# hip-satomi/microbeSEG

Measured on AMD Instinct MI355X. Metric: training crops/sec (256px), higher is better.
Workload: dtype f32; 1 GPU; BASELINE configs[1]: DU-Net distance-map training step, filters [64, 1024], 256x256 crops, per-GPU batch 32, fp32, relu/bn, SmoothL1x2 + Adam(amsgrad); global_batch=32, parallelism=dp1, launch=eager

## Files before the change

### include/mseg_hip.h

```cpp
#ifndef MSEG_HIP_H
#define MSEG_HIP_H

#include <stddef.h>
#include <stdint.h>

#ifdef __cplusplus
extern "C" {
#endif

#define MSEG_OK 0
#define MSEG_EINVAL (-1)
#define MSEG_ELAUNCH (-2)
#define MSEG_EWORKSPACE (-3)

#define MSEG_ACT_NONE 0
#define MSEG_ACT_RELU 1
#define MSEG_ACT_LEAKY 2
#define MSEG_ACT_ELU 3
#define MSEG_ACT_MISH 4

#define MSEG_NORM_BN 0
#define MSEG_NORM_GN 1
#define MSEG_NORM_IN 2

// ... 5 lines not shown
  const float* shift;
  int32_t C;
  int32_t act;
  int32_t ss;
  int32_t dtype;
} MsegSrc;

#define MSEG_MODE_CONV 0
#define MSEG_MODE_TCONV 1
#define MSEG_EPI_PLAIN 0
#define MSEG_EPI_SCATTER2X2 1
#define MSEG_MORDER_LINEAR 0
#define MSEG_MORDER_PARITY 1
#define MSEG_PREC_F32 0
#define MSEG_PREC_BF16 1

typedef struct MsegIgemm {
  MsegSrc src[2];
  const float* w;
  const float* bias;
  float* dst0;
  float* dst1;
  int32_t nsrc, Cin, Kpad, Npad;
  int32_t NB, Hi, Wi, Ho, Wo;
  int32_t KH, KW, stride, pad, mode, morder;
  int32_t Ngemm, epi, split, ld0, ld1, acc0, acc1, Cq;
  int32_t precision;
  int32_t dst_dtype;
  void* ws;
  size_t ws_bytes;
  float* stats;
  int32_t stats_act;
  int32_t reserved0;
} MsegIgemm;

int mseg_igemm(const MsegIgemm* p, void* stream);

typedef struct MsegKernelInfo {
  char name[120];
  int32_t precision;
  int32_t launches;
  uint32_t grid, block;
  size_t workspace;
  int32_t stats_rows;
  int32_t reserved0;
} MsegKernelInfo;
int mseg_igemm_query(const MsegIgemm* p, MsegKernelInfo* info);
const char* mseg_last_kernel(void);
int mseg_f32_to_bf16(const float* src, uint16_t* dst, size_t n, void* stream);
size_t mseg_igemm_workspace_bytes(const MsegIgemm* p);
int mseg_igemm_set_persistent(int on);
int mseg_igemm_set_wide_tiles(int on);
int mseg_igemm_set_p8(int mode);

typedef struct MsegWgrad {
  MsegSrc P;
  MsegSrc Q[2];
  float* ws;
  float* dst;
  int32_t nq, Nch, Nch_store;
  int32_t NB, Hp, Wp, Hq, Wq;
  int32_t KH, KW, stride, pad;
  int32_t splits;
  int32_t phase;
  int32_t precision;
  int32_t reserved;
} MsegWgrad;
// ... 176 lines not shown
```

### microbeseg_amd/_lib.py

```python
import ctypes as C
import os
import pathlib

_HERE = pathlib.Path(__file__).resolve().parent
LIB_PATH = _HERE / "libmseg_hip.so"

ACT = {"none": 0, "relu": 1, "leakyrelu": 2, "elu": 3, "mish": 4}
NORM = {"bn": 0, "gn": 1, "in": 2}
MODE_CONV, MODE_TCONV = 0, 1
EPI_PLAIN, EPI_SCATTER2X2 = 0, 1
MORDER_LINEAR, MORDER_PARITY = 0, 1
ST_F32, ST_BF16 = 0, 1


class MsegLibraryError(RuntimeError):
    pass


class MsegSrc(C.Structure):
    _fields_ = [("ptr", C.c_void_p), ("scale", C.c_void_p), ("shift", C.c_void_p),
                ("C", C.c_int32), ("act", C.c_int32), ("ss", C.c_int32), ("dtype", C.c_int32)]


class MsegIgemm(C.Structure):
    _fields_ = [("src", MsegSrc * 2), ("w", C.c_void_p), ("bias", C.c_void_p), ("dst0", C.c_void_p),
                ("dst1", C.c_void_p),
                ("nsrc", C.c_int32), ("Cin", C.c_int32), ("Kpad", C.c_int32), ("Npad", C.c_int32),
                ("NB", C.c_int32), ("Hi", C.c_int32), ("Wi", C.c_int32), ("Ho", C.c_int32), ("Wo", C.c_int32),
                ("KH", C.c_int32), ("KW", C.c_int32), ("stride", C.c_int32), ("pad", C.c_int32),
                ("mode", C.c_int32), ("morder", C.c_int32),
                ("Ngemm", C.c_int32), ("epi", C.c_int32), ("split", C.c_int32), ("ld0", C.c_int32),
                ("ld1", C.c_int32), ("acc0", C.c_int32), ("acc1", C.c_int32), ("Cq", C.c_int32),
                ("precision", C.c_int32), ("dst_dtype", C.c_int32), ("ws", C.c_void_p), ("ws_bytes", C.c_size_t),
                ("stats", C.c_void_p), ("stats_act", C.c_int32), ("reserved0", C.c_int32)]


class MsegWgrad(C.Structure):
    _fields_ = [("P", MsegSrc), ("Q", MsegSrc * 2), ("ws", C.c_void_p), ("dst", C.c_void_p),
                ("nq", C.c_int32), ("Nch", C.c_int32), ("Nch_store", C.c_int32),
                ("NB", C.c_int32), ("Hp", C.c_int32), ("Wp", C.c_int32), ("Hq", C.c_int32), ("Wq", C.c_int32),
                ("KH", C.c_int32), ("KW", C.c_int32), ("stride", C.c_int32), ("pad", C.c_int32),
                ("splits", C.c_int32), ("phase", C.c_int32), ("precision", C.c_int32), ("reserved", C.c_int32)]


class MsegKernelInfo(C.Structure):
    _fields_ = [("name", C.c_char * 120), ("precision", C.c_int32), ("launches", C.c_int32), ("grid", C.c_uint32),
                ("block", C.c_uint32), ("workspace", C.c_size_t), ("stats_rows", C.c_int32), ("reserved0", C.c_int32)]


class MsegPackJob(C.Structure):
    _fields_ = [("src", C.c_void_p), ("dst", C.c_void_p), ("dst16", C.c_void_p),
                ("T", C.c_int32), ("R", C.c_int32), ("Rpad", C.c_int32), ("C", C.c_int32), ("Cpad", C.c_int32),
                ("st", C.c_int32), ("sr", C.c_int32), ("sc", C.c_int32),
                ("first_block", C.c_uint32), ("reserved", C.c_uint32)]


class MsegRangerJob(C.Structure):
    _fields_ = [("p", C.c_void_p), ("g", C.c_void_p), ("m", C.c_void_p), ("v", C.c_void_p), ("slow", C.c_void_p),
                ("n", C.c_uint64), ("rows", C.c_int32), ("step_lr", C.c_float), ("flags", C.c_uint32),
                ("reserved", C.c_uint32)]


_P = C.c_void_p
_I = C.c_int
_F = C.c_float
_D = C.c_double
_SZ = C.c_size_t
# ... 127 lines not shown
```

### microbeseg_amd/csrc/igemm.hip

```cpp
#include "common.h"
#include "igemm_common.h"
#include "bf16_affine.h"

int igemm_p8_try(const MsegIgemm& p, int tr, int m_fastest, int cus, hipStream_t st);

__device__ float g_ident_scale[MSEG_MAX_CH];
__device__ float g_ident_shift[MSEG_MAX_CH];
__global__ void init_ident_kernel() {
  for (int i = blockIdx.x * blockDim.x + threadIdx.x; i < MSEG_MAX_CH; i += gridDim.x * blockDim.x) {
    g_ident_scale[i] = 1.f;
    g_ident_shift[i] = 0.f;
  }
}


template <int BM, int BN, bool PER_SAMPLE, bool GENERIC_ACT>
__global__ __launch_bounds__(256) void igemm_kernel(const MsegIgemm p) {
  using Cfg = IgemmCfg<BM, BN>;
  constexpr int STAGE = (BM + BN) * LDS_STRIDE;
  __shared__ __attribute__((aligned(16))) float lds[2 * STAGE + 4];
  unsigned* tapmask_s = reinterpret_cast<unsigned*>(lds + 2 * STAGE);

  const int tid = threadIdx.x;
  const int lane = tid & 63;
  const int wave = tid >> 6;
  const int wm = wave / Cfg::WN, wn = wave % Cfg::WN;

  const int M = p.NB * p.Ho * p.Wo;
  const int ntiles_n = (p.Ngemm + BN - 1) / BN;
  const int lid = (int)xcd_logical_id(blockIdx.x, gridDim.x);
  const int tile_m = lid / ntiles_n;
  const int tile_n = lid - tile_m * ntiles_n;
  const int m0 = tile_m * BM, n0 = tile_n * BN;

  const int T = p.KH * p.KW;
  const int srow = tid >> 3;
  const int scol = tid & 7;
// ... 169 lines not shown
#pragma unroll
        for (int b = 0; b < Cfg::NB; ++b) {
          acc[a][b] = __builtin_amdgcn_mfma_f32_32x32x2f32(af[a].x, bf[b].x, acc[a][b], 0, 0, 0);
          acc[a][b] = __builtin_amdgcn_mfma_f32_32x32x2f32(af[a].y, bf[b].y, acc[a][b], 0, 0, 0);
          acc[a][b] = __builtin_amdgcn_mfma_f32_32x32x2f32(af[a].z, bf[b].z, acc[a][b], 0, 0, 0);
          acc[a][b] = __builtin_amdgcn_mfma_f32_32x32x2f32(af[a].w, bf[b].w, acc[a][b], 0, 0, 0);
        }
    }
    float* An = lds + (cur ^ 1) * STAGE;
#ifdef MSEG_ABLATE
    STAMP(s2);
    if (!(abl & 8)) commit(An, An + BM * LDS_STRIDE);
    STAMP(s3);
    if (!(abl & 2)) __syncthreads();
    STAMP(s4);
    t_issue += s1 - s0; t_mfma += s2 - s1; t_commit += s3 - s2; t_bar += s4 - s3;
#else
    commit(An, An + BM * LDS_STRIDE);
    __syncthreads();
#endif
    cur ^= 1;
    have = have_next;
  }

#ifdef MSEG_ABLATE
  if ((abl & 32) && p.dst1 && lane == 0 && blockIdx.x < 1024) {
    float* dbg = p.dst1 + ((size_t)blockIdx.x * 4 + wave) * 4;
    dbg[0] = (float)t_issue; dbg[1] = (float)t_mfma; dbg[2] = (float)t_commit; dbg[3] = (float)t_bar;
  }
#endif
  igemm_epilogue<IgemmCfg<BM, BN>>(acc, m0, n0, wm, wn, lane, M);
}

template <int BM, int BN, int TR, bool PER_SAMPLE, bool SB = false>
__global__ __launch_bounds__(256) void igemm_fast_kernel(const MsegIgemm p) {
  using Cfg = IgemmCfg<BM, BN>;
  constexpr int STAGE = (BM + BN) * LDS_STRIDE;
  __shared__ __attribute__((aligned(16))) float lds[(SB ? 1 : 2) * STAGE];

  const int tid = threadIdx.x;
  const int lane = tid & 63;
  const int wave = tid >> 6;
  const int wm = wave / Cfg::WN, wn = wave % Cfg::WN;
  const int M = p.NB * p.Ho * p.Wo;
  const int ntiles_n = (p.Ngemm + BN - 1) / BN;
  const int lid = (int)xcd_logical_id(blockIdx.x, gridDim.x);
  const int tile_m = lid / ntiles_n;
  const int tile_n = lid - tile_m * ntiles_n;
  const int m0 = tile_m * BM, n0 = tile_n * BN;
  const int T = p.KH * p.KW;
  const int srow = tid >> 3, scol = tid & 7;

  const TapGeom geom = make_geom(p);
  const long long tile_px = tile_base_pixel(p, geom, m0, M);
  int pix0[Cfg::AROWS];
  int rown[Cfg::AROWS];
  unsigned vmask[Cfg::AROWS];
#pragma unroll
  for (int i = 0; i < Cfg::AROWS; ++i) {
    const RowInfo r = decode_row(p, m0 + srow + 32 * i, M);
    const int iy0 = (r.oy * geom.sm - geom.dir * geom.pad) >> geom.sh, ix0 = (r.ox * geom.sm - geom.dir * geom.pad) >> geom.sh;
    pix0[i] = (int)(((long long)r.n * p.Hi + iy0) * p.Wi + ix0 - tile_px);
    rown[i] = r.n < 0 ? 0 : r.n;
    unsigned mk = 0u;
    for (int t = 0; t < T; ++t) {
      const int ky = t / p.KW, kx = t - ky * p.KW;
      int iy, ix;
      mk |= (unsigned)tap_coord(geom, r, ky, kx, iy, ix) << t;
    }
    vmask[i] = mk;
  }

  f32x16 acc[Cfg::MB][Cfg::NB];
#pragma unroll
  for (int a = 0; a < Cfg::MB; ++a)
#pragma unroll
    for (int b = 0; b < Cfg::NB; ++b)
#pragma unroll
      for (int r = 0; r < 16; ++r) acc[a][b][r] = 0.f;

  const int nchunks = (p.Cin + KC - 1) / KC;
  const int C0 = p.src[0].C;
  const unsigned OOB = 0x80000000u;

  const __amdgpu_buffer_rsrc_t rs0 = __builtin_amdgcn_make_buffer_rsrc(
      const_cast<float*>(p.src[0].ptr + tile_px * p.src[0].C), 0, 0x7ffffff0, 0x00020000);
  const __amdgpu_buffer_rsrc_t rs1 = __builtin_amdgcn_make_buffer_rsrc(
      const_cast<float*>((p.nsrc > 1 ? p.src[1].ptr : p.src[0].ptr) + tile_px * (p.nsrc > 1 ? p.src[1].C : p.src[0].C)), 0,
      0x7ffffff0, 0x00020000);
  const __amdgpu_buffer_rsrc_t rsw = __builtin_amdgcn_make_buffer_rsrc(const_cast<float*>(p.w), 0,
                                                                        T * p.Npad * p.Kpad * 4, 0x00020000);
  unsigned wvoff[Cfg::BROWS];
#pragma unroll
  for (int i = 0; i < Cfg::BROWS; ++i) wvoff[i] = ((unsigned)(n0 + srow + 32 * i) * (unsigned)p.Kpad + scol * 4u) * 4u;

  constexpr int NSC = (TR == 0) ? 1 : (PER_SAMPLE ? Cfg::AROWS : 1);
  float4 ra[Cfg::AROWS], rb[Cfg::BROWS], rsc[NSC], rsh[NSC];
  float rm[Cfg::AROWS];
  unsigned rowoff[Cfg::AROWS];
  int ract = 0;
  int cur_chunk = -1;
  bool cur_s1 = false;

  auto issue = [&](int chunk, int t, int ky, int kx) {
    const int c = chunk * KC + scol * 4;
    if (chunk != cur_chunk) {
      cur_chunk = chunk;
      cur_s1 = (p.nsrc > 1) && (chunk * KC >= C0);
      const unsigned sC4 = (unsigned)(cur_s1 ? p.src[1].C : p.src[0].C) * 4u;
      const unsigned cl4 = (unsigned)(cur_s1 ? c - C0 : c) * 4u;
#pragma unroll
      for (int i = 0; i < Cfg::AROWS; ++i) rowoff[i] = (unsigned)pix0[i] * sC4 + cl4;
      if (TR != 0) {
        const MsegSrc& s = cur_s1 ? p.src[1] : p.src[0];
        ract = s.act;
        const bool has_aff = s.scale != nullptr;
        const float* scp = has_aff ? s.scale : g_ident_scale;
        const float* shp = has_aff ? s.shift : g_ident_shift;
        const unsigned cl = (c < p.Cin) ? (cl4 >> 2) : 0u;
#pragma unroll
        for (int i = 0; i < NSC; ++i) {
          const size_t o = (size_t)(PER_SAMPLE ? rown[i] : 0) * (has_aff ? (unsigned)s.ss : 0u) + cl;
          rsc[i] = *reinterpret_cast<const float4*>(scp + o);
          rsh[i] = *reinterpret_cast<const float4*>(shp + o);
        }
      }
    }
// ... 3 lines not shown
#pragma unroll
    for (int i = 0; i < Cfg::AROWS; ++i) {
      const bool ok = (vmask[i] & cbit) != 0u;
      const unsigned vo = ok ? rowoff[i] + delta : OOB;
      const f32x4 v = cur_s1 ? __builtin_bit_cast(f32x4, __builtin_amdgcn_raw_buffer_load_b128(rs1, vo, 0, 0))
                             : __builtin_bit_cast(f32x4, __builtin_amdgcn_raw_buffer_load_b128(rs0, vo, 0, 0));
      ra[i] = make_float4(v[0], v[1], v[2], v[3]);
      if (TR != 0) rm[i] = ok ? 1.f : 0.f;
    }
    const unsigned wso = ((unsigned)t * (unsigned)p.Npad * (unsigned)p.Kpad + (unsigned)chunk * KC) * 4u;
#pragma unroll
    for (int i = 0; i < Cfg::BROWS; ++i) {
      const f32x4 v = __builtin_bit_cast(f32x4, __builtin_amdgcn_raw_buffer_load_b128(rsw, wvoff[i], wso, 0));
      rb[i] = make_float4(v[0], v[1], v[2], v[3]);
    }
  };

  auto commit = [&](float* As, float* Bs) {
    const float lo = (ract == MSEG_ACT_RELU) ? 0.f : -3.402823466e38f;
#pragma unroll
    for (int i = 0; i < Cfg::AROWS; ++i) {
      float4 v = ra[i];
      if (TR != 0) {
        if (TR == 2) {
          v = act_fwd4(v, ract);
        } else {
          v.x = clamp_lo(v.x, lo); v.y = clamp_lo(v.y, lo); v.z = clamp_lo(v.z, lo); v.w = clamp_lo(v.w, lo);
        }
        const float4 sc = rsc[PER_SAMPLE ? i : 0], sh = rsh[PER_SAMPLE ? i : 0];
        const float m = rm[i];
        v.x = (v.x * sc.x + sh.x) * m; v.y = (v.y * sc.y + sh.y) * m;
        v.z = (v.z * sc.z + sh.z) * m; v.w = (v.w * sc.w + sh.w) * m;
      }
      *reinterpret_cast<float4*>(As + (srow + 32 * i) * LDS_STRIDE + scol * 4) = v;
    }
#pragma unroll
    for (int i = 0; i < Cfg::BROWS; ++i)
      *reinterpret_cast<float4*>(Bs + (srow + 32 * i) * LDS_STRIDE + scol * 4) = rb[i];
  };

  unsigned long long taplist = 0ull, taplist_hi = 0ull;
  int nlive = 0;
  {
    int py = 0, px = 0;
    if (geom.sh) {
      const int cls = m0 / (M >> 2);
      py = cls >> 1; px = cls & 1;
    }
    for (int tt = 0; tt < T; ++tt) {
      const int ky_ = tt / p.KW, kx_ = tt - ky_ * p.KW;
      const bool live = (((py - geom.dir * (ky_ - geom.pad)) | (px - geom.dir * (kx_ - geom.pad))) & geom.sh) == 0;
      if (live) {
        const unsigned long long e = (unsigned long long)(tt | (ky_ << 4) | (kx_ << 6));
        if (nlive < 8) taplist |= e << (8 * nlive); else taplist_hi |= e << (8 * (nlive - 8));
        ++nlive;
      }
    }
  }
  auto tap_at = [&](int j) -> unsigned { return (unsigned)((j < 8 ? taplist >> (8 * j) : taplist_hi >> (8 * (j - 8))) & 0xffull); };
  int chunk = 0, j = 0;
  const int nsteps = nchunks * nlive;
  unsigned e0 = tap_at(0);
  issue(0, (int)(e0 & 15u), (int)((e0 >> 4) & 3u), (int)(e0 >> 6));
  commit(lds, lds + BM * LDS_STRIDE);
  __syncthreads();
  int cur = 0;
  const int li = lane & 31, lh = lane >> 5;
  for (int step = 0; step < nsteps; ++step) {
    if (step + 1 < nsteps) {
      j += 1;
      if (j >= nlive) { j = 0; ++chunk; }
    }
    e0 = tap_at(j);
    issue(chunk, (int)(e0 & 15u), (int)((e0 >> 4) & 3u), (int)(e0 >> 6));

    const float* As = lds + cur * STAGE;
    const float* Bs = As + BM * LDS_STRIDE;
#pragma unroll
    for (int kk = 0; kk < KC / 8; ++kk) {
      float4 af[Cfg::MB], bf[Cfg::NB];
#pragma unroll
      for (int a = 0; a < Cfg::MB; ++a)
        af[a] = *reinterpret_cast<const float4*>(As + (wm * Cfg::TM + a * 32 + li) * LDS_STRIDE + kk * 8 + lh * 4);
#pragma unroll
      for (int b = 0; b < Cfg::NB; ++b)
        bf[b] = *reinterpret_cast<const float4*>(Bs + (wn * Cfg::TN + b * 32 + li) * LDS_STRIDE + kk * 8 + lh * 4);
#pragma unroll
      for (int a = 0; a < Cfg::MB; ++a)
#pragma unroll
        for (int b = 0; b < Cfg::NB; ++b) {
          acc[a][b] = __builtin_amdgcn_mfma_f32_32x32x2f32(af[a].x, bf[b].x, acc[a][b], 0, 0, 0);
          acc[a][b] = __builtin_amdgcn_mfma_f32_32x32x2f32(af[a].y, bf[b].y, acc[a][b], 0, 0, 0);
          acc[a][b] = __builtin_amdgcn_mfma_f32_32x32x2f32(af[a].z, bf[b].z, acc[a][b], 0, 0, 0);
          acc[a][b] = __builtin_amdgcn_mfma_f32_32x32x2f32(af[a].w, bf[b].w, acc[a][b], 0, 0, 0);
        }
    }
    if (SB) {
      __syncthreads();
      commit(lds, lds + BM * LDS_STRIDE);
      __syncthreads();
    } else {
      float* An = lds + (cur ^ 1) * STAGE;
      commit(An, An + BM * LDS_STRIDE);
      __syncthreads();
      cur ^= 1;
    }
  }
  igemm_epilogue<IgemmCfg<BM, BN>>(acc, m0, n0, wm, wn, lane, M);
}

template <int BN>
struct HaloCfg {
  static constexpr int WN = (BN >= 128) ? 4 : 2;
  static constexpr int WM = 8 / WN;
  static constexpr int TM = 128 / WM, TN = BN / WN;
  static constexpr int MB = TM / 32, NB = TN / 32;
  static constexpr int BROWS = BN / 64;
};

template <int BN, int TR>
__global__ __launch_bounds__(512, 2) void igemm_halo_kernel(const MsegIgemm p, int tw_log2, int ksplit,
                                                            int chunks_per_split) {
  constexpr int BM = 128;
  using Cfg = HaloCfg<BN>;
  constexpr int HMAX = 264;
  constexpr int HL = (HMAX * 8 + 511) / 512;
  constexpr int ASTAGE = HMAX * LDS_STRIDE;
  constexpr int BSTAGE = BN * LDS_STRIDE;
  __shared__ __attribute__((aligned(16))) float lds[ASTAGE + 2 * BSTAGE];
  float* const Abuf = lds;
  float* const Bbuf = lds + ASTAGE;

  const int tid = threadIdx.x, lane = tid & 63, wave = tid >> 6;
  const int wm = wave / Cfg::WN, wn = wave % Cfg::WN;
  const int li = lane & 31, lh = lane >> 5;
  const int srow = tid >> 3, scol = tid & 7;
  const int TW = 1 << tw_log2, TH = BM >> tw_log2, HW2 = TW + 2;
  const int HROWS = (TH + 2) * HW2;
  const int H = p.Hi, W = p.Wi;
  const int M = p.NB * H * W;
  const int tiles_x = W >> tw_log2, tiles_y = (H + TH - 1) / TH;
// ... 2159 lines not shown
    return MSEG_OK;
  }
  if (p.precision == MSEG_PREC_BF16 && s16 && g_c64p_on && plain && p.epi == MSEG_EPI_PLAIN && p.KH == 2 && p.KW == 2 &&
      p.stride == 2 && p.pad == 0 && p.mode == MSEG_MODE_CONV && p.morder == MSEG_MORDER_LINEAR && p.nsrc == 1 &&
      p.Cin == 64 && p.Kpad == 64 && p.Ngemm == 128 && p.split >= p.Ngemm && !p.acc0 && !p.bias && (p.Wo % 32) == 0 &&
      p.Hi == 2 * p.Ho && p.Wi == 2 * p.Wo && (M % 64) == 0 && M / 64 >= 4 * (long long)c64p_workgroups()) {
    const dim3 pgrid((unsigned)c64p_workgroups());
    if (p.dst_dtype == MSEG_ST_BF16) MSEG_KL((igemm_ctd_bf16_kernel<true>), pgrid, dim3(512), 0, st, p, (int)(M / 64));
    else MSEG_KL((igemm_ctd_bf16_kernel<false>), pgrid, dim3(512), 0, st, p, (int)(M / 64));
    MSEG_LAUNCH_CHECK();
    return MSEG_OK;
  }
  if (p.precision == MSEG_PREC_BF16) {
    if (!fast) return MSEG_EINVAL;
    const int tr = plain ? 0 : (generic ? 2 : 1);
#define MSEG_FAST16_LAUNCH(BM_, BN_, TR_, PS_)                                                          \
  do {                                                                                                  \
    if (s16) MSEG_KL((igemm_fast_bf16_kernel<BM_, BN_, TR_, PS_, true>), grid, block, 0, st, p);   \
    else MSEG_KL((igemm_fast_bf16_kernel<BM_, BN_, TR_, PS_, false>), grid, block, 0, st, p);      \
  } while (0)
#define MSEG_FAST16_TILE(BM_, BN_)                                                        \
  do {                                                                                    \
    if (tr == 0) MSEG_FAST16_LAUNCH(BM_, BN_, 0, false);                                  \
    else if (tr == 1) { if (per_sample) MSEG_FAST16_LAUNCH(BM_, BN_, 1, true); else MSEG_FAST16_LAUNCH(BM_, BN_, 1, false); } \
    else { if (per_sample) MSEG_FAST16_LAUNCH(BM_, BN_, 2, true); else MSEG_FAST16_LAUNCH(BM_, BN_, 2, false); }              \
  } while (0)
    if (wide) MSEG_FAST16_TILE(128, 128); else MSEG_FAST16_TILE(128, 64);
#undef MSEG_FAST16_TILE
#undef MSEG_FAST16_LAUNCH
    MSEG_LAUNCH_CHECK();
    return MSEG_OK;
  }
  if (fast) {
    const int tr = plain ? 0 : (generic ? 2 : 1);
    const int live_taps = (p.mode == MSEG_MODE_TCONV && p.stride == 2) ? ((p.KH + 1) / 2) * ((p.KW + 1) / 2) : p.KH * p.KW;
    const bool short_k = ((p.Cin + KC - 1) / KC) * live_taps <= 8;
#define MSEG_FAST_LAUNCH(BM_, BN_, TR_, PS_)                                                              \
  do {                                                                                                    \
    if (short_k) MSEG_KL((igemm_fast_kernel<BM_, BN_, TR_, PS_, true>), grid, block, 0, st, p); \
    else MSEG_KL((igemm_fast_kernel<BM_, BN_, TR_, PS_, false>), grid, block, 0, st, p);        \
  } while (0)
#define MSEG_FAST_TILE(BM_, BN_)                                                          \
  do {                                                                                    \
    if (tr == 0) MSEG_FAST_LAUNCH(BM_, BN_, 0, false);                                    \
    else if (tr == 1) { if (per_sample) MSEG_FAST_LAUNCH(BM_, BN_, 1, true); else MSEG_FAST_LAUNCH(BM_, BN_, 1, false); } \
    else { if (per_sample) MSEG_FAST_LAUNCH(BM_, BN_, 2, true); else MSEG_FAST_LAUNCH(BM_, BN_, 2, false); }              \
  } while (0)
    if (wide) MSEG_FAST_TILE(128, 128); else MSEG_FAST_TILE(128, 64);
#undef MSEG_FAST_TILE
#undef MSEG_FAST_LAUNCH
    MSEG_LAUNCH_CHECK();
    return MSEG_OK;
  }
#define MSEG_IGEMM_LAUNCH(BM_, BN_, PS_, GA_) \
  MSEG_KL((igemm_kernel<BM_, BN_, PS_, GA_>), grid, block, 0, st, p)
  if (wide) {
    if (per_sample) { if (generic) MSEG_IGEMM_LAUNCH(128, 128, true, true); else MSEG_IGEMM_LAUNCH(128, 128, true, false); }
    else            { if (generic) MSEG_IGEMM_LAUNCH(128, 128, false, true); else MSEG_IGEMM_LAUNCH(128, 128, false, false); }
  } else {
    if (per_sample) { if (generic) MSEG_IGEMM_LAUNCH(128, 64, true, true); else MSEG_IGEMM_LAUNCH(128, 64, true, false); }
    else            { if (generic) MSEG_IGEMM_LAUNCH(128, 64, false, true); else MSEG_IGEMM_LAUNCH(128, 64, false, false); }
  }
#undef MSEG_IGEMM_LAUNCH
  MSEG_LAUNCH_CHECK();
  return MSEG_OK;
}

extern "C" int mseg_igemm(const MsegIgemm* pp, void* stream) {
  mseg_dispatch_begin(0);
  const int rc = igemm_dispatch(pp, stream);
  mseg_dispatch_end(nullptr);
  return rc;
}

// ... 99 lines not shown
```

### microbeseg_amd/engine.py

```python
import ctypes as C
import os

import torch

from . import _lib
from ._lib import (ACT, NORM, MODE_CONV, MODE_TCONV, EPI_PLAIN, EPI_SCATTER2X2, MORDER_LINEAR, MORDER_PARITY,
                   ST_F32, ST_BF16, MsegSrc, MsegIgemm, MsegWgrad, MsegKernelInfo, check)

BN_EPS = 1e-5
BN_MOMENTUM = 0.1


def _ptr(t):
    return None if t is None else t.data_ptr()


def _stream():
    return torch.cuda.current_stream().cuda_stream


def _pad4(c):
    return (c + 3) // 4 * 4


# ... 329 lines not shown
    __slots__ = ("name", "bf16", "launches", "grid", "block", "workspace", "stats_rows")

    def __init__(self, info):
        self.name = info.name.decode()
        self.bf16 = info.precision == 1
        self.launches, self.grid, self.block, self.workspace = info.launches, info.grid, info.block, info.workspace
        self.stats_rows = info.stats_rows

    def __repr__(self):
        return f"KernelChoice({self.name!r}, bf16={self.bf16}, grid={self.grid})"


def _fill_igemm(p, srcs, kpad, npad, NB, Hi, Wi, Ho, Wo, KH, KW, stride, pad, mode, Ngemm, ld0, acc0, ld1, acc1, split, epi,
                Cq, morder):
    for i, s in enumerate(srcs):
        p.src[i] = s
    p.nsrc = len(srcs)
    p.Cin = sum(s.C for s in srcs)
    p.Kpad, p.Npad = kpad, npad
    p.NB, p.Hi, p.Wi, p.Ho, p.Wo = NB, Hi, Wi, Ho, Wo
    p.KH, p.KW, p.stride, p.pad, p.mode, p.morder = KH, KW, stride, pad, mode, morder
    p.Ngemm, p.epi = Ngemm, epi
    p.split = Ngemm if split is None else split
    p.ld0, p.ld1, p.acc0, p.acc1, p.Cq = ld0, ld1, acc0, acc1, Cq


def _query(fn, p):
    info = MsegKernelInfo()
    rc = fn(C.byref(p), C.byref(info))
    return KernelChoice(info) if rc == 0 else None


def igemm_query(srcs, kpad, npad, NB, Hi, Wi, Ho, Wo, KH, KW, stride, pad, mode, Ngemm, ld0, acc0=0, ld1=0, acc1=0,
                split=None, epi=EPI_PLAIN, Cq=0, morder=MORDER_LINEAR, precision=None, dst_dtype=ST_F32, bias=True):
    p = MsegIgemm()
    _fill_igemm(p, srcs, kpad, npad, NB, Hi, Wi, Ho, Wo, KH, KW, stride, pad, mode, Ngemm, ld0, acc0, ld1, acc1, split, epi, Cq,
                morder)
    p.w = p.dst0 = _DUMMY
    p.dst1 = _DUMMY if (split is not None and split < Ngemm) else None
    p.bias = _DUMMY if bias else None
    p.precision = 1 if (precision or _precision) == "bf16" else 0
    p.dst_dtype = dst_dtype
    return _query(_lib.load().mseg_igemm_query, p)


_bf16_ok_cache = {}


def _igemm_bf16_ok(p):
    key = (p.nsrc, tuple((p.src[i].C, p.src[i].act, bool(p.src[i].scale), p.src[i].ss != 0, p.src[i].dtype)
                         for i in range(p.nsrc)), p.Kpad, p.Npad, p.NB, p.Hi, p.Wi, p.Ho, p.Wo, p.KH, p.KW, p.stride, p.pad,
           p.mode, p.morder, p.Ngemm, p.epi, p.split, p.ld0, p.ld1, p.acc0, p.acc1, p.Cq, p.dst_dtype, bool(p.bias))
    ok = _bf16_ok_cache.get(key)
    if ok is None:
        p.precision = 1
        ok = _bf16_ok_cache[key] = _query(_lib.load().mseg_igemm_query, p) is not None
    return ok


_conv_stats = os.environ.get("MSEG_CONV_STATS", "0") == "1"


def set_conv_stats(flag):
    global _conv_stats
    old, _conv_stats = _conv_stats, bool(flag)
    return old


def igemm(srcs, w, bias, NB, Hi, Wi, Ho, Wo, KH, KW, stride, pad, mode, Ngemm, dst0, ld0, acc0=0,
          dst1=None, ld1=0, acc1=0, split=None, epi=EPI_PLAIN, Cq=0, morder=MORDER_LINEAR, real_cin=None,
          precision=None, stats=None):
    lib = _lib.load()
    p = MsegIgemm()
    _fill_igemm(p, srcs, w.Kpad, w.Npad, NB, Hi, Wi, Ho, Wo, KH, KW, stride, pad, mode, Ngemm, ld0, acc0, ld1, acc1, split, epi,
                Cq, morder)
    p.w = w.t.data_ptr()
    p.dst_dtype = _st(dst0)
    p.bias = _ptr(bias)
    p.dst0 = dst0.data_ptr()
    p.dst1 = _ptr(dst1)
    bf16 = (precision or _precision) == "bf16" and _igemm_bf16_ok(p)
    if bf16:
        p.w = w.bf16().data_ptr()
    p.precision = 1 if bf16 else 0
    need = lib.mseg_igemm_workspace_bytes(C.byref(p))
    if need:
        key = (dst0.device, _stream())
        buf = _splitk_ws.get(key)
        if buf is None or buf.numel() < need:
            buf = torch.empty(need, dtype=torch.uint8, device=dst0.device)
            _splitk_ws[key] = buf
        p.ws, p.ws_bytes = buf.data_ptr(), buf.numel()
    taken = None
    if stats is not None and bf16 and _conv_stats:
        p.stats, p.stats_act = _DUMMY, stats[0]
        choice = _query(lib.mseg_igemm_query, p)
        rows = choice.stats_rows if choice else 0
        if rows > 0:
            part = stats[1].get("convstats", rows * 2 * Ngemm * 4)
            p.stats = part.data_ptr()
            taken = (part, rows)
        else:
            p.stats = None
    if _timer is None:
        check(lib.mseg_igemm(C.byref(p), _stream()), "igemm")
        return taken
    flops = 2.0 * NB * Ho * Wo * Ngemm * (p.Cin if real_cin is None else real_cin) * KH * KW
    if mode == MODE_TCONV:
# ... 634 lines not shown
```

### microbeseg_amd/csrc/igemm_common.h

```cpp
#pragma once
#include "common.h"

#define KC 32
#define LDS_STRIDE 36
#define MSEG_MAX_CH 8192

template <int BM, int BN>
struct IgemmCfg {
  static constexpr int WM = (BN >= 128) ? 2 : 4;
  static constexpr int WN = 4 / WM;
  static constexpr int TM = BM / WM;
  static constexpr int TN = BN / WN;
  static constexpr int MB = TM / 32;
  static constexpr int NB = TN / 32;
  static constexpr int AROWS = BM / 32;
  static constexpr int BROWS = BN / 32;
};

struct RowInfo {
  int n;
  int oy, ox;
};

__device__ __forceinline__ RowInfo decode_row(const MsegIgemm& p, int m, int M) {
  RowInfo r;
  if (m >= M) { r.n = -1; r.oy = 0; r.ox = 0; return r; }
  if (p.morder == MSEG_MORDER_PARITY) {
    const int Hh = p.Ho >> 1, Wh = p.Wo >> 1;
    const int per = p.NB * Hh * Wh;
    const int cls = m / per;
    int rem = m - cls * per;
    r.n = rem / (Hh * Wh);
    rem -= r.n * (Hh * Wh);
    const int y2 = rem / Wh;
    r.oy = 2 * y2 + (cls >> 1);
    r.ox = 2 * (rem - y2 * Wh) + (cls & 1);
  } else {
    r.n = m / (p.Ho * p.Wo);
    int rem = m - r.n * (p.Ho * p.Wo);
    r.oy = rem / p.Wo;
    r.ox = rem - r.oy * p.Wo;
  }
  return r;
}

struct TapGeom { int sm, dir, sh, pad, Hi, Wi; };

__device__ __forceinline__ TapGeom make_geom(const MsegIgemm& p) {
  TapGeom g;
// ... 181 lines not shown
```

Before: 245.0 crops/s.

## Add 512-thread 8-wave igemm kernel for stride-2 conv and transposed-conv paths

Adds a new f32 implicit-GEMM kernel with 8 waves per block (BM=128) and a precomputed live-tap list. It is used for 3x3 stride-2 conv-pool, 1x1 scatter transposed-conv forward and 2x2 stride-2 dgrad shapes, and takes priority over the existing fast kernel unless a new `kernel` field forces FAST. Per-row tap validity is precomputed as masks and loads go through buffer resources with OOB offsets to avoid branches. The aim is better MFMA utilization and latency hiding on these down/up-sampling layers. The risks are register pressure at two blocks of 512 threads and a struct ABI change.

```diff
diff --git a/include/mseg_hip.h b/include/mseg_hip.h
--- a/include/mseg_hip.h
+++ b/include/mseg_hip.h
@@ -61,7 +61,11 @@
   float* stats;
   int32_t stats_act;
   int32_t reserved0;
+  int32_t kernel;
+  int32_t reserved1;
 } MsegIgemm;
+#define MSEG_IGEMM_KERNEL_AUTO 0
+#define MSEG_IGEMM_KERNEL_FAST 1
 
 int mseg_igemm(const MsegIgemm* p, void* stream);
 
diff --git a/microbeseg_amd/_lib.py b/microbeseg_amd/_lib.py
--- a/microbeseg_amd/_lib.py
+++ b/microbeseg_amd/_lib.py
@@ -32,7 +32,8 @@
                 ("Ngemm", C.c_int32), ("epi", C.c_int32), ("split", C.c_int32), ("ld0", C.c_int32),
                 ("ld1", C.c_int32), ("acc0", C.c_int32), ("acc1", C.c_int32), ("Cq", C.c_int32),
                 ("precision", C.c_int32), ("dst_dtype", C.c_int32), ("ws", C.c_void_p), ("ws_bytes", C.c_size_t),
-                ("stats", C.c_void_p), ("stats_act", C.c_int32), ("reserved0", C.c_int32)]
+                ("stats", C.c_void_p), ("stats_act", C.c_int32), ("reserved0", C.c_int32),
+                ("kernel", C.c_int32), ("reserved1", C.c_int32)]
 
 
 class MsegWgrad(C.Structure):
diff --git a/microbeseg_amd/csrc/igemm.hip b/microbeseg_amd/csrc/igemm.hip
--- a/microbeseg_amd/csrc/igemm.hip
+++ b/microbeseg_amd/csrc/igemm.hip
@@ -3,6 +3,7 @@
 #include "bf16_affine.h"
 
 int igemm_p8_try(const MsegIgemm& p, int tr, int m_fastest, int cus, hipStream_t st);
+int igemm_s2_try(const MsegIgemm& p, int tr, bool per_sample, hipStream_t st);
 
 __device__ float g_ident_scale[MSEG_MAX_CH];
 __device__ float g_ident_shift[MSEG_MAX_CH];
@@ -2668,6 +2669,10 @@
     return MSEG_OK;
   }
   if (fast) {
+    const int rc = igemm_s2_try(p, plain ? 0 : (generic ? 2 : 1), per_sample, st);
+    if (rc != 0) return rc < 0 ? rc : MSEG_OK;
+  }
+  if (fast) {
     const int tr = plain ? 0 : (generic ? 2 : 1);
     const int live_taps = (p.mode == MSEG_MODE_TCONV && p.stride == 2) ? ((p.KH + 1) / 2) * ((p.KW + 1) / 2) : p.KH * p.KW;
     const bool short_k = ((p.Cin + KC - 1) / KC) * live_taps <= 8;
diff --git a/microbeseg_amd/csrc/igemm_s2.hip b/microbeseg_amd/csrc/igemm_s2.hip
--- /dev/null
+++ b/microbeseg_amd/csrc/igemm_s2.hip
@@ -0,0 +1,246 @@
+#include "common.h"
+#include "igemm_common.h"
+
+template <int BM, int BN>
+struct IgemmCfg8 {
+  static constexpr int WM = (BN >= 128) ? 2 : 4;
+  static constexpr int WN = 8 / WM;
+  static constexpr int TM = BM / WM;
+  static constexpr int TN = BN / WN;
+  static constexpr int MB = TM / 32;
+  static constexpr int NB = TN / 32;
+  static constexpr int AROWS = BM / 64;
+  static constexpr int BROWS = BN / 64;
+};
+template <int BN, int TR, bool PER_SAMPLE>
+__global__ __launch_bounds__(512, 2) void igemm_s2_kernel(const MsegIgemm p) {
+  constexpr int BM = 128;
+  using Cfg = IgemmCfg8<BM, BN>;
+  constexpr int STAGE = (BM + BN) * LDS_STRIDE;
+  __shared__ __attribute__((aligned(16))) float lds[2 * STAGE];
+
+  const int tid = threadIdx.x;
+  const int lane = tid & 63;
+  const int wave = tid >> 6;
+  const int wm = wave / Cfg::WN, wn = wave % Cfg::WN;
+  const int M = p.NB * p.Ho * p.Wo;
+  const int ntiles_n = (p.Ngemm + BN - 1) / BN;
+  const int lid = (int)xcd_logical_id(blockIdx.x, gridDim.x);
+  const int tile_m = lid / ntiles_n;
+  const int tile_n = lid - tile_m * ntiles_n;
+  const int m0 = tile_m * BM, n0 = tile_n * BN;
+  const int T = p.KH * p.KW;
+  const int srow = tid >> 3, scol = tid & 7;
+
+  const TapGeom geom = make_geom(p);
+  const long long tile_px = tile_base_pixel(p, geom, m0, M);
+  int pix0[Cfg::AROWS];
+  int rown[Cfg::AROWS];
+  unsigned vmask[Cfg::AROWS];
+#pragma unroll
+  for (int i = 0; i < Cfg::AROWS; ++i) {
+    const RowInfo r = decode_row(p, m0 + srow + 64 * i, M);
+    const int iy0 = (r.oy * geom.sm - geom.dir * geom.pad) >> geom.sh, ix0 = (r.ox * geom.sm - geom.dir * geom.pad) >> geom.sh;
+    pix0[i] = (int)(((long long)r.n * p.Hi + iy0) * p.Wi + ix0 - tile_px);
+    rown[i] = r.n < 0 ? 0 : r.n;
+    unsigned mk = 0u;
+    for (int t = 0; t < T; ++t) {
+      const int ky = t / p.KW, kx = t - ky * p.KW;
+      int iy, ix;
+      mk |= (unsigned)tap_coord(geom, r, ky, kx, iy, ix) << t;
+    }
+    vmask[i] = mk;
+  }
+
+  f32x16 acc[Cfg::MB][Cfg::NB];
+#pragma unroll
+  for (int a = 0; a < Cfg::MB; ++a)
+#pragma unroll
+    for (int b = 0; b < Cfg::NB; ++b)
+#pragma unroll
+      for (int r = 0; r < 16; ++r) acc[a][b][r] = 0.f;
+
+  const int nchunks = (p.Cin + KC - 1) / KC;
+  const int C0 = p.src[0].C;
+  const unsigned OOB = 0x80000000u;
+
+  const __amdgpu_buffer_rsrc_t rs0 = __builtin_amdgcn_make_buffer_rsrc(
+      const_cast<float*>(p.src[0].ptr + tile_px * p.src[0].C), 0, 0x7ffffff0, 0x00020000);
+  const __amdgpu_buffer_rsrc_t rs1 = __builtin_amdgcn_make_buffer_rsrc(
+      const_cast<float*>((p.nsrc > 1 ? p.src[1].ptr : p.src[0].ptr) + tile_px * (p.nsrc > 1 ? p.src[1].C : p.src[0].C)), 0,
+      0x7ffffff0, 0x00020000);
+  const __amdgpu_buffer_rsrc_t rsw = __builtin_amdgcn_make_buffer_rsrc(const_cast<float*>(p.w), 0,
+                                                                        T * p.Npad * p.Kpad * 4, 0x00020000);
+  unsigned wvoff[Cfg::BROWS];
+#pragma unroll
+  for (int i = 0; i < Cfg::BROWS; ++i) wvoff[i] = ((unsigned)(n0 + srow + 64 * i) * (unsigned)p.Kpad + scol * 4u) * 4u;
+
+  constexpr int NSC = (TR == 0) ? 1 : (PER_SAMPLE ? Cfg::AROWS : 1);
+  float4 ra[Cfg::AROWS], rb[Cfg::BROWS], rsc[NSC], rsh[NSC];
+  float rm[Cfg::AROWS];
+  unsigned rowoff[Cfg::AROWS];
+  int ract = 0;
+  int cur_chunk = -1;
+  bool cur_s1 = false;
+
+  auto issue = [&](int chunk, int t, int ky, int kx) {
+    const int c = chunk * KC + scol * 4;
+    if (chunk != cur_chunk) {
+      cur_chunk = chunk;
+      cur_s1 = (p.nsrc > 1) && (chunk * KC >= C0);
+      const unsigned sC4 = (unsigned)(cur_s1 ? p.src[1].C : p.src[0].C) * 4u;
+      const unsigned cl4 = (unsigned)(cur_s1 ? c - C0 : c) * 4u;
+#pragma unroll
+      for (int i = 0; i < Cfg::AROWS; ++i) rowoff[i] = (unsigned)pix0[i] * sC4 + cl4;
+      if (TR != 0) {
+        const MsegSrc& s = cur_s1 ? p.src[1] : p.src[0];
+        ract = s.act;
+        if (s.scale != nullptr) {
+          const unsigned cl = (c < p.Cin) ? (cl4 >> 2) : 0u;
+#pragma unroll
+          for (int i = 0; i < NSC; ++i) {
+            const size_t o = (size_t)(PER_SAMPLE ? rown[i] : 0) * (unsigned)s.ss + cl;
+            rsc[i] = *reinterpret_cast<const float4*>(s.scale + o);
+            rsh[i] = *reinterpret_cast<const float4*>(s.shift + o);
+          }
+        } else {
+#pragma unroll
+          for (int i = 0; i < NSC; ++i) {
+            rsc[i] = make_float4(1.f, 1.f, 1.f, 1.f);
+            rsh[i] = make_float4(0.f, 0.f, 0.f, 0.f);
+          }
+        }
+      }
+    }
+    const unsigned cbit = (c < p.Cin) ? (1u << t) : 0u;
+    const unsigned sC4 = (unsigned)(cur_s1 ? p.src[1].C : p.src[0].C) * 4u;
+    const unsigned delta = (unsigned)(geom.dir * ((ky >> geom.sh) * p.Wi + (kx >> geom.sh))) * sC4;
+#pragma unroll
+    for (int i = 0; i < Cfg::AROWS; ++i) {
+      const bool ok = (vmask[i] & cbit) != 0u;
+      const unsigned vo = ok ? rowoff[i] + delta : OOB;
+      const f32x4 v = cur_s1 ? __builtin_bit_cast(f32x4, __builtin_amdgcn_raw_buffer_load_b128(rs1, vo, 0, 0))
+                             : __builtin_bit_cast(f32x4, __builtin_amdgcn_raw_buffer_load_b128(rs0, vo, 0, 0));
+      ra[i] = make_float4(v[0], v[1], v[2], v[3]);
+      if (TR != 0) rm[i] = ok ? 1.f : 0.f;
+    }
+    const unsigned wso = ((unsigned)t * (unsigned)p.Npad * (unsigned)p.Kpad + (unsigned)chunk * KC) * 4u;
+#pragma unroll
+    for (int i = 0; i < Cfg::BROWS; ++i) {
+      const f32x4 v = __builtin_bit_cast(f32x4, __builtin_amdgcn_raw_buffer_load_b128(rsw, wvoff[i], wso, 0));
+      rb[i] = make_float4(v[0], v[1], v[2], v[3]);
+    }
+  };
+
+  auto commit = [&](float* As, float* Bs) {
+    const float lo = (ract == MSEG_ACT_RELU) ? 0.f : -3.402823466e38f;
+#pragma unroll
+    for (int i = 0; i < Cfg::AROWS; ++i) {
+      float4 v = ra[i];
+      if (TR != 0) {
+        if (TR == 2) {
+          v = act_fwd4(v, ract);
+        } else {
+          v.x = clamp_lo(v.x, lo); v.y = clamp_lo(v.y, lo); v.z = clamp_lo(v.z, lo); v.w = clamp_lo(v.w, lo);
+        }
+        const float4 sc = rsc[PER_SAMPLE ? i : 0], sh = rsh[PER_SAMPLE ? i : 0];
+        const float m = rm[i];
+        v.x = (v.x * sc.x + sh.x) * m; v.y = (v.y * sc.y + sh.y) * m;
+        v.z = (v.z * sc.z + sh.z) * m; v.w = (v.w * sc.w + sh.w) * m;
+      }
+      *reinterpret_cast<float4*>(As + (srow + 64 * i) * LDS_STRIDE + scol * 4) = v;
+    }
+#pragma unroll
+    for (int i = 0; i < Cfg::BROWS; ++i)
+      *reinterpret_cast<float4*>(Bs + (srow + 64 * i) * LDS_STRIDE + scol * 4) = rb[i];
+  };
+
+  unsigned long long taplist = 0ull, taplist_hi = 0ull;
+  int nlive = 0;
+  {
+    int py = 0, px = 0;
+    if (geom.sh) {
+      const int cls = m0 / (M >> 2);
+      py = cls >> 1; px = cls & 1;
+    }
+    for (int tt = 0; tt < T; ++tt) {
+      const int ky_ = tt / p.KW, kx_ = tt - ky_ * p.KW;
+      const bool live = (((py - geom.dir * (ky_ - geom.pad)) | (px - geom.dir * (kx_ - geom.pad))) & geom.sh) == 0;
+      if (live) {
+        const unsigned long long e = (unsigned long long)(tt | (ky_ << 4) | (kx_ << 6));
+        if (nlive < 8) taplist |= e << (8 * nlive); else taplist_hi |= e << (8 * (nlive - 8));
+        ++nlive;
+      }
+    }
+  }
+  auto tap_at = [&](int j) -> unsigned { return (unsigned)((j < 8 ? taplist >> (8 * j) : taplist_hi >> (8 * (j - 8))) & 0xffull); };
+  int chunk = 0, j = 0;
+  const int nsteps = nchunks * nlive;
+  unsigned e0 = tap_at(0);
+  issue(0, (int)(e0 & 15u), (int)((e0 >> 4) & 3u), (int)(e0 >> 6));
+  commit(lds, lds + BM * LDS_STRIDE);
+  __syncthreads();
+  int cur = 0;
+  const int li = lane & 31, lh = lane >> 5;
+  for (int step = 0; step < nsteps; ++step) {
+    if (step + 1 < nsteps) {
+      j += 1;
+      if (j >= nlive) { j = 0; ++chunk; }
+    }
+    e0 = tap_at(j);
+    issue(chunk, (int)(e0 & 15u), (int)((e0 >> 4) & 3u), (int)(e0 >> 6));
+
+    const float* As = lds + cur * STAGE;
+    const float* Bs = As + BM * LDS_STRIDE;
+#pragma unroll
+    for (int kk = 0; kk < KC / 8; ++kk) {
+      float4 af[Cfg::MB], bf[Cfg::NB];
+#pragma unroll
+      for (int a = 0; a < Cfg::MB; ++a)
+        af[a] = *reinterpret_cast<const float4*>(As + (wm * Cfg::TM + a * 32 + li) * LDS_STRIDE + kk * 8 + lh * 4);
+#pragma unroll
+      for (int b = 0; b < Cfg::NB; ++b)
+        bf[b] = *reinterpret_cast<const float4*>(Bs + (wn * Cfg::TN + b * 32 + li) * LDS_STRIDE + kk * 8 + lh * 4);
+#pragma unroll
+      for (int a = 0; a < Cfg::MB; ++a)
+#pragma unroll
+        for (int b = 0; b < Cfg::NB; ++b) {
+          acc[a][b] = __builtin_amdgcn_mfma_f32_32x32x2f32(af[a].x, bf[b].x, acc[a][b], 0, 0, 0);
+          acc[a][b] = __builtin_amdgcn_mfma_f32_32x32x2f32(af[a].y, bf[b].y, acc[a][b], 0, 0, 0);
+          acc[a][b] = __builtin_amdgcn_mfma_f32_32x32x2f32(af[a].z, bf[b].z, acc[a][b], 0, 0, 0);
+          acc[a][b] = __builtin_amdgcn_mfma_f32_32x32x2f32(af[a].w, bf[b].w, acc[a][b], 0, 0, 0);
+        }
+    }
+    float* An = lds + (cur ^ 1) * STAGE;
+    commit(An, An + BM * LDS_STRIDE);
+    __syncthreads();
+    cur ^= 1;
+  }
+  igemm_epilogue<Cfg>(acc, m0, n0, wm, wn, lane, M);
+}
+
+int igemm_s2_try(const MsegIgemm& p, int tr, bool per_sample, hipStream_t st) {
+  if (p.precision != MSEG_PREC_F32 || p.kernel == MSEG_IGEMM_KERNEL_FAST) return 0;
+  const bool convpool = p.KH == 3 && p.KW == 3 && p.stride == 2 && p.pad == 1;
+  const bool ct_fwd = p.epi == MSEG_EPI_SCATTER2X2 && p.KH == 1 && p.KW == 1 && p.stride == 1 && p.pad == 0 &&
+                      p.mode == MSEG_MODE_CONV;
+  const bool ct_dgrad = p.KH == 2 && p.KW == 2 && p.stride == 2 && p.pad == 0 && p.mode == MSEG_MODE_CONV;
+  if (!convpool && !ct_fwd && !ct_dgrad) return 0;
+  for (int i = 0; i < p.nsrc; ++i)
+    if ((long long)p.NB * p.Hi * p.Wi * p.src[i].C * 4 >= 0x80000000LL) return 0;
+  const long long M = (long long)p.NB * p.Ho * p.Wo;
+  const int BN = p.Ngemm > 64 ? 128 : 64;
+  const dim3 grid((unsigned)(((M + 127) / 128) * ((p.Ngemm + BN - 1) / BN))), block(512);
+#define MSEG_S2_LAUNCH(BN_, TR_, PS_) MSEG_KL((igemm_s2_kernel<BN_, TR_, PS_>), grid, block, 0, st, p)
+#define MSEG_S2_TILE(BN_)                                                                                       \
+  do {                                                                                                          \
+    if (tr == 0) MSEG_S2_LAUNCH(BN_, 0, false);                                                                 \
+    else if (tr == 1) { if (per_sample) MSEG_S2_LAUNCH(BN_, 1, true); else MSEG_S2_LAUNCH(BN_, 1, false); }     \
+    else { if (per_sample) MSEG_S2_LAUNCH(BN_, 2, true); else MSEG_S2_LAUNCH(BN_, 2, false); }                  \
+  } while (0)
+  if (BN == 128) MSEG_S2_TILE(128); else MSEG_S2_TILE(64);
+#undef MSEG_S2_TILE
+#undef MSEG_S2_LAUNCH
+  MSEG_LAUNCH_CHECK();
+  return 1;
+}
diff --git a/microbeseg_amd/engine.py b/microbeseg_amd/engine.py
--- a/microbeseg_amd/engine.py
+++ b/microbeseg_amd/engine.py
@@ -385,10 +385,12 @@
 
 
 def igemm_query(srcs, kpad, npad, NB, Hi, Wi, Ho, Wo, KH, KW, stride, pad, mode, Ngemm, ld0, acc0=0, ld1=0, acc1=0,
-                split=None, epi=EPI_PLAIN, Cq=0, morder=MORDER_LINEAR, precision=None, dst_dtype=ST_F32, bias=True):
+                split=None, epi=EPI_PLAIN, Cq=0, morder=MORDER_LINEAR, precision=None, dst_dtype=ST_F32, bias=True,
+                kernel=0):
     p = MsegIgemm()
     _fill_igemm(p, srcs, kpad, npad, NB, Hi, Wi, Ho, Wo, KH, KW, stride, pad, mode, Ngemm, ld0, acc0, ld1, acc1, split, epi, Cq,
                 morder)
+    p.kernel = kernel
     p.w = p.dst0 = _DUMMY
     p.dst1 = _DUMMY if (split is not None and split < Ngemm) else None
     p.bias = _DUMMY if bias else None
@@ -422,11 +424,12 @@
 
 def igemm(srcs, w, bias, NB, Hi, Wi, Ho, Wo, KH, KW, stride, pad, mode, Ngemm, dst0, ld0, acc0=0,
           dst1=None, ld1=0, acc1=0, split=None, epi=EPI_PLAIN, Cq=0, morder=MORDER_LINEAR, real_cin=None,
-          precision=None, stats=None):
+          precision=None, stats=None, kernel=0):
     lib = _lib.load()
     p = MsegIgemm()
     _fill_igemm(p, srcs, w.Kpad, w.Npad, NB, Hi, Wi, Ho, Wo, KH, KW, stride, pad, mode, Ngemm, ld0, acc0, ld1, acc1, split, epi,
                 Cq, morder)
+    p.kernel = kernel
     p.w = w.t.data_ptr()
     p.dst_dtype = _st(dst0)
     p.bias = _ptr(bias)
```

New measurement: 245.4 crops/s (median of 6 runs). About the same (+0.2%).

## Run fast implicit-GEMM with 8-wave blocks and remap transposed-conv tile order

Applied to the files above, without the earlier changes.

Widens the fast implicit-GEMM kernel from 4 to 8 waves per block (512 threads, launch bounds for 2 blocks per CU). The wave grid and row pitch are generalised through a new NW parameter in IgemmCfg. It drops the single-buffered short-K variant so every shape uses the double-buffered LDS pipeline. For stride-2 transposed convs it also remaps block-to-tile order across the parity classes and XCDs to balance live-tap work. The aim is more MFMA work and latency hiding per block, at the cost of register pressure and possible bad tilings for small BM/BN, where per-wave tiles could shrink to zero.

```diff
diff --git a/microbeseg_amd/csrc/igemm.hip b/microbeseg_amd/csrc/igemm.hip
--- a/microbeseg_amd/csrc/igemm.hip
+++ b/microbeseg_amd/csrc/igemm.hip
@@ -238,11 +238,11 @@
   igemm_epilogue<IgemmCfg<BM, BN>>(acc, m0, n0, wm, wn, lane, M);
 }
 
-template <int BM, int BN, int TR, bool PER_SAMPLE, bool SB = false>
-__global__ __launch_bounds__(256) void igemm_fast_kernel(const MsegIgemm p) {
-  using Cfg = IgemmCfg<BM, BN>;
+template <int BM, int BN, int TR, bool PER_SAMPLE>
+__global__ __launch_bounds__(512, 2) void igemm_fast_kernel(const MsegIgemm p) {
+  using Cfg = IgemmCfg<BM, BN, 8>;
   constexpr int STAGE = (BM + BN) * LDS_STRIDE;
-  __shared__ __attribute__((aligned(16))) float lds[(SB ? 1 : 2) * STAGE];
+  __shared__ __attribute__((aligned(16))) float lds[2 * STAGE];
 
   const int tid = threadIdx.x;
   const int lane = tid & 63;
@@ -251,20 +251,32 @@
   const int M = p.NB * p.Ho * p.Wo;
   const int ntiles_n = (p.Ngemm + BN - 1) / BN;
   const int lid = (int)xcd_logical_id(blockIdx.x, gridDim.x);
-  const int tile_m = lid / ntiles_n;
-  const int tile_n = lid - tile_m * ntiles_n;
+  int tile_m = lid / ntiles_n;
+  int tile_n = lid - tile_m * ntiles_n;
+  const TapGeom geom = make_geom(p);
+  if (geom.sh) {
+    const int tpc = (M >> 2) / BM;
+    if ((tpc & 1) == 0) {
+      const int g = (int)(blockIdx.x >> 3), xcd = (int)(blockIdx.x & 7u);
+      const int ml = g / ntiles_n;
+      tile_n = g - ml * ntiles_n;
+      const int o = ml * 8 + xcd, oc = o / tpc;
+      tile_m = (3 - oc) * tpc + (o - oc * tpc);
+    } else {
+      tile_m = (tile_m & 3) * tpc + (tile_m >> 2);
+    }
+  }
   const int m0 = tile_m * BM, n0 = tile_n * BN;
   const int T = p.KH * p.KW;
   const int srow = tid >> 3, scol = tid & 7;
 
-  const TapGeom geom = make_geom(p);
   const long long tile_px = tile_base_pixel(p, geom, m0, M);
   int pix0[Cfg::AROWS];
   int rown[Cfg::AROWS];
   unsigned vmask[Cfg::AROWS];
 #pragma unroll
   for (int i = 0; i < Cfg::AROWS; ++i) {
-    const RowInfo r = decode_row(p, m0 + srow + 32 * i, M);
+    const RowInfo r = decode_row(p, m0 + srow + Cfg::RP * i, M);
     const int iy0 = (r.oy * geom.sm - geom.dir * geom.pad) >> geom.sh, ix0 = (r.ox * geom.sm - geom.dir * geom.pad) >> geom.sh;
     pix0[i] = (int)(((long long)r.n * p.Hi + iy0) * p.Wi + ix0 - tile_px);
     rown[i] = r.n < 0 ? 0 : r.n;
@@ -298,7 +310,7 @@
                                                                         T * p.Npad * p.Kpad * 4, 0x00020000);
   unsigned wvoff[Cfg::BROWS];
 #pragma unroll
-  for (int i = 0; i < Cfg::BROWS; ++i) wvoff[i] = ((unsigned)(n0 + srow + 32 * i) * (unsigned)p.Kpad + scol * 4u) * 4u;
+  for (int i = 0; i < Cfg::BROWS; ++i) wvoff[i] = ((unsigned)(n0 + srow + Cfg::RP * i) * (unsigned)p.Kpad + scol * 4u) * 4u;
 
   constexpr int NSC = (TR == 0) ? 1 : (PER_SAMPLE ? Cfg::AROWS : 1);
   float4 ra[Cfg::AROWS], rb[Cfg::BROWS], rsc[NSC], rsh[NSC];
@@ -368,11 +380,11 @@
         v.x = (v.x * sc.x + sh.x) * m; v.y = (v.y * sc.y + sh.y) * m;
         v.z = (v.z * sc.z + sh.z) * m; v.w = (v.w * sc.w + sh.w) * m;
       }
-      *reinterpret_cast<float4*>(As + (srow + 32 * i) * LDS_STRIDE + scol * 4) = v;
+      *reinterpret_cast<float4*>(As + (srow + Cfg::RP * i) * LDS_STRIDE + scol * 4) = v;
     }
 #pragma unroll
     for (int i = 0; i < Cfg::BROWS; ++i)
-      *reinterpret_cast<float4*>(Bs + (srow + 32 * i) * LDS_STRIDE + scol * 4) = rb[i];
+      *reinterpret_cast<float4*>(Bs + (srow + Cfg::RP * i) * LDS_STRIDE + scol * 4) = rb[i];
   };
 
   unsigned long long taplist = 0ull, taplist_hi = 0ull;
@@ -431,18 +443,12 @@
           acc[a][b] = __builtin_amdgcn_mfma_f32_32x32x2f32(af[a].w, bf[b].w, acc[a][b], 0, 0, 0);
         }
     }
-    if (SB) {
-      __syncthreads();
-      commit(lds, lds + BM * LDS_STRIDE);
-      __syncthreads();
-    } else {
-      float* An = lds + (cur ^ 1) * STAGE;
-      commit(An, An + BM * LDS_STRIDE);
-      __syncthreads();
-      cur ^= 1;
-    }
-  }
-  igemm_epilogue<IgemmCfg<BM, BN>>(acc, m0, n0, wm, wn, lane, M);
+    float* An = lds + (cur ^ 1) * STAGE;
+    commit(An, An + BM * LDS_STRIDE);
+    __syncthreads();
+    cur ^= 1;
+  }
+  igemm_epilogue<Cfg>(acc, m0, n0, wm, wn, lane, M);
 }
 
 template <int BN>
@@ -2669,13 +2675,8 @@
   }
   if (fast) {
     const int tr = plain ? 0 : (generic ? 2 : 1);
-    const int live_taps = (p.mode == MSEG_MODE_TCONV && p.stride == 2) ? ((p.KH + 1) / 2) * ((p.KW + 1) / 2) : p.KH * p.KW;
-    const bool short_k = ((p.Cin + KC - 1) / KC) * live_taps <= 8;
-#define MSEG_FAST_LAUNCH(BM_, BN_, TR_, PS_)                                                              \
-  do {                                                                                                    \
-    if (short_k) MSEG_KL((igemm_fast_kernel<BM_, BN_, TR_, PS_, true>), grid, block, 0, st, p); \
-    else MSEG_KL((igemm_fast_kernel<BM_, BN_, TR_, PS_, false>), grid, block, 0, st, p);        \
-  } while (0)
+    const dim3 block8(512);
+#define MSEG_FAST_LAUNCH(BM_, BN_, TR_, PS_) MSEG_KL((igemm_fast_kernel<BM_, BN_, TR_, PS_>), grid, block8, 0, st, p)
 #define MSEG_FAST_TILE(BM_, BN_)                                                          \
   do {                                                                                    \
     if (tr == 0) MSEG_FAST_LAUNCH(BM_, BN_, 0, false);                                    \
diff --git a/microbeseg_amd/csrc/igemm_common.h b/microbeseg_amd/csrc/igemm_common.h
--- a/microbeseg_amd/csrc/igemm_common.h
+++ b/microbeseg_amd/csrc/igemm_common.h
@@ -5,16 +5,17 @@
 #define LDS_STRIDE 36
 #define MSEG_MAX_CH 8192
 
-template <int BM, int BN>
+template <int BM, int BN, int NW = 4>
 struct IgemmCfg {
-  static constexpr int WM = (BN >= 128) ? 2 : 4;
-  static constexpr int WN = 4 / WM;
+  static constexpr int WN = (BN >= 128) ? NW / 2 : NW / 4;
+  static constexpr int WM = NW / WN;
   static constexpr int TM = BM / WM;
   static constexpr int TN = BN / WN;
   static constexpr int MB = TM / 32;
   static constexpr int NB = TN / 32;
-  static constexpr int AROWS = BM / 32;
-  static constexpr int BROWS = BN / 32;
+  static constexpr int RP = NW * 8;
+  static constexpr int AROWS = BM / RP;
+  static constexpr int BROWS = BN / RP;
 };
 
 struct RowInfo {
```

Measured after the change: 243.4 crops/s before, 245.9 crops/s after, median of 6. No clear change (+1.0%).
